# AvalonEnjoyer/pytorch-ViT-paper-replication

Measured on AMD Instinct MI355X. Metric: images/sec (whole node) ViT-B/16 224px bf16 at 1/2/4/8 MI355X, higher is better.
Workload: dtype bf16; 1 GPU; model=ViT-B/16, global_batch=256, per_gpu_batch=256, seq_len=197, image_size=224, parallelism=dp1, impl=fused, grad_transport=none, optimizer=Adam(wd=0.03 decay group) + clip 1.0 + warmup/linear-decay LR, dropout=0.1 (mlp, embedding)

## Files before the change

pytorch_vit_paper_replication_amd/csrc/attention.hip:

```cpp
#include "attn_common.h"
#include "kernels.h"

namespace pvr {
namespace {


template <int DH, bool DROP, int QG, int KT>
__global__ void __launch_bounds__(256) __attribute__((amdgpu_waves_per_eu(3))) attn_fwd_kernel(const uint16_t* __restrict__ qkv, int64_t ld, uint16_t* __restrict__ out,
                                                        int64_t ld_o, float* __restrict__ lse, int N, int H, int D, float scale,
                                                        AttnDrop drop, AttnQ8 q8) {
  using C = Hd<DH>;
  static_assert(KT == 32 || KT == 64, "keys per tile");
  constexpr int NFR = KT / 16;
  constexpr int TILE_BYTES = KT * 128 * C::NH;
  constexpr int QW = 16 * QG;
  extern __shared__ __attribute__((aligned(16))) char smem[];
  const int lane = threadIdx.x & 63;
  const int wave = __builtin_amdgcn_readfirstlane(threadIdx.x >> 6);
  const int g = lane >> 4, li = lane & 15;
  const int nqb = (N + 4 * QW - 1) / (4 * QW);
  const int L = xcd_remap(blockIdx.x, gridDim.x);
  const int bh = L / nqb, b = bh / H, h = bh % H;
  const int q0 = (L % nqb) * 4 * QW + wave * QW;

// ... 1760 lines not shown
}
PVR_DEV uint4 cls_pack8(const float (&f)[8]) {
  return make_uint4(pack2bf(f[0], f[1]), pack2bf(f[2], f[3]), pack2bf(f[4], f[5]), pack2bf(f[6], f[7]));
}
PVR_DEV float cls_dot8(const float (&a)[8], const float (&b)[8]) {
  float s = 0.f;
#pragma unroll
  for (int j = 0; j < 8; ++j) s = fmaf(a[j], b[j], s);
  return s;
}
template <int CH>
PVR_DEV float cls_group_sum(float v, int gbase) {
  if constexpr (CH == 8) {
    return oct_sum(v);
  } else if constexpr (CH == 16) {
    return row16_sum(v);
  } else {
    float t = 0.f;
#pragma unroll
    for (int j = 0; j < CH; ++j) t += __shfl(v, min(gbase + j, 63), 64);
    return t;
  }
}
template <bool MAX>
PVR_DEV float cls_block_reduce(float v, float* r4) {
  v = MAX ? wave_max(v) : wave_sum(v);
  __syncthreads();
  if ((threadIdx.x & 63) == 0) r4[threadIdx.x >> 6] = v;
  __syncthreads();
  return MAX ? fmaxf(fmaxf(r4[0], r4[1]), fmaxf(r4[2], r4[3])) : (r4[0] + r4[1]) + (r4[2] + r4[3]);
}

template <int DH>
__global__ void __launch_bounds__(256) attn_cls_fwd_kernel(const uint16_t* __restrict__ qkv, int64_t ld, uint16_t* __restrict__ out,
                                                            int64_t ld_o, float* __restrict__ lse, int N, int H, int D, float scale) {
  constexpr int CH = DH / 8, GPW = 64 / CH, NG = 4 * GPW;
  extern __shared__ float cls_sc[];
  __shared__ float gred[NG * DH];
  __shared__ float r4[4];
  const int bh = blockIdx.x, b = bh / H, h = bh % H;
  const int tid = threadIdx.x, lane = tid & 63, wave = tid >> 6;
  const int g = lane / CH, c = lane % CH;
  const bool act = g < GPW;
  const uint16_t* base = qkv + (int64_t)b * N * ld + h * DH + c * 8;
  float qf[8];
#pragma unroll
  for (int j = 0; j < 8; ++j) qf[j] = 0.f;
  if (act) cls_unpack8(*(const uint4*)base, qf);
  for (int k0 = wave * GPW; k0 < N; k0 += NG) {
    const int k = k0 + g;
    const bool live = act && k < N;
    float sv = 0.f;
    if (live) {
      float kf[8];
      cls_unpack8(*(const uint4*)(base + (int64_t)k * ld + D), kf);
      sv = cls_dot8(qf, kf);
    }
    sv = cls_group_sum<CH>(sv, g * CH);
    if (live && c == 0) cls_sc[k] = sv * scale;
  }
  __syncthreads();
  float m = -INFINITY;
  for (int k = tid; k < N; k += 256) m = fmaxf(m, cls_sc[k]);
  m = cls_block_reduce<true>(m, r4);
  float l = 0.f;
  for (int k = tid; k < N; k += 256) {
    const float pk = __builtin_amdgcn_exp2f((cls_sc[k] - m) * LOG2E);
    cls_sc[k] = pk;
    l += pk;
  }
  l = cls_block_reduce<false>(l, r4);
  if (tid == 0) lse[bh] = m + logf(l);
  float acc[8];
#pragma unroll
  for (int j = 0; j < 8; ++j) acc[j] = 0.f;
  if (act) {
    for (int k = wave * GPW + g; k < N; k += NG) {
      float vf[8];
      cls_unpack8(*(const uint4*)(base + (int64_t)k * ld + 2 * D), vf);
      const float pk = cls_sc[k];
#pragma unroll
      for (int j = 0; j < 8; ++j) acc[j] = fmaf(pk, vf[j], acc[j]);
    }
#pragma unroll
    for (int j = 0; j < 8; ++j) gred[(wave * GPW + g) * DH + c * 8 + j] = acc[j];
  }
  __syncthreads();
  if (tid < DH) {
    float o = 0.f;
#pragma unroll 4
    for (int gg = 0; gg < NG; ++gg) o += gred[gg * DH + tid];
    out[(int64_t)b * ld_o + h * DH + tid] = f2bf(o / l);
  }
}

template <int DH>
__global__ void __launch_bounds__(256) attn_cls_bwd_kernel(const uint16_t* __restrict__ qkv, int64_t ld, const uint16_t* __restrict__ o,
                                                            int64_t ld_o, const uint16_t* __restrict__ dout, int64_t ld_do,
                                                            const float* __restrict__ lse, uint16_t* __restrict__ dqkv, int64_t ld_dq,
                                                            float* __restrict__ dq0, int N, int H, int D, float scale) {
  constexpr int CH = DH / 8, GPW = 64 / CH, NG = 4 * GPW;
  __shared__ float gred[NG * DH];
  const int bh = blockIdx.x, b = bh / H, h = bh % H;
  const int tid = threadIdx.x, lane = tid & 63, wave = tid >> 6;
  const int g = lane / CH, c = lane % CH;
  const bool act = g < GPW;
  const int col = h * DH + c * 8;
  const uint16_t* base = qkv + (int64_t)b * N * ld + col;
  uint16_t* dbase = dqkv + (int64_t)b * N * ld_dq + col;
  float qf[8], dof[8], dqa[8];
#pragma unroll
  for (int j = 0; j < 8; ++j) qf[j] = dof[j] = dqa[j] = 0.f;
  float dpart = 0.f;
  if (act) {
    float of[8];
    cls_unpack8(*(const uint4*)base, qf);
    cls_unpack8(*(const uint4*)(dout + (int64_t)b * ld_do + col), dof);
    cls_unpack8(*(const uint4*)(o + (int64_t)b * ld_o + col), of);
    dpart = cls_dot8(dof, of);
  }
  const float delta = cls_group_sum<CH>(dpart, g * CH);
  const float l2 = lse[bh] * LOG2E, sl2 = scale * LOG2E;
  for (int k0 = wave * GPW; k0 < N; k0 += NG) {
    const int k = k0 + g;
    const bool live = act && k < N;
    float kf[8], vf[8];
    float sv = 0.f, tv = 0.f;
    if (live) {
      const uint4 kq = *(const uint4*)(base + (int64_t)k * ld + D);
      const uint4 vq = *(const uint4*)(base + (int64_t)k * ld + 2 * D);
      cls_unpack8(kq, kf);
      cls_unpack8(vq, vf);
      sv = cls_dot8(qf, kf);
      tv = cls_dot8(dof, vf);
    }
    sv = cls_group_sum<CH>(sv, g * CH);
    tv = cls_group_sum<CH>(tv, g * CH);
    if (live) {
      const float pk = __builtin_amdgcn_exp2f(sv * sl2 - l2);
      const float ds = pk * (tv - delta) * scale;
      float dk[8], dv[8];
#pragma unroll
      for (int j = 0; j < 8; ++j) {
        dv[j] = pk * dof[j];
        dk[j] = ds * qf[j];
        dqa[j] = fmaf(ds, kf[j], dqa[j]);
      }
      uint16_t* row = dbase + (int64_t)k * ld_dq;
      if (k > 0) *(uint4*)row = make_uint4(0u, 0u, 0u, 0u);
      *(uint4*)(row + D) = cls_pack8(dk);
      *(uint4*)(row + 2 * D) = cls_pack8(dv);
    }
  }
  if (act) {
#pragma unroll
    for (int j = 0; j < 8; ++j) gred[(wave * GPW + g) * DH + c * 8 + j] = dqa[j];
  }
  __syncthreads();
  if (tid < DH) {
    float dq = 0.f;
#pragma unroll 4
    for (int gg = 0; gg < NG; ++gg) dq += gred[gg * DH + tid];
    dqkv[(int64_t)b * N * ld_dq + h * DH + tid] = f2bf(dq);
    dq0[(int64_t)b * D + h * DH + tid] = dq;
  }
}

__global__ void __launch_bounds__(256) attn_cls_dbias_kernel(const float* __restrict__ dq0, const uint16_t* __restrict__ dout,
                                                              int64_t ld_do, float* __restrict__ dbias, int B, int D) {
  const int col = blockIdx.x * 256 + threadIdx.x;
  if (col >= D) return;
  float sq = 0.f, sv = 0.f;
#pragma unroll 8
  for (int b = 0; b < B; ++b) {
    sq += dq0[(int64_t)b * D + col];
    sv += bf2f(dout[(int64_t)b * ld_do + col]);
  }
  dbias[col] += sq;
  dbias[2 * D + col] += sv;
}

bool attn_cls_args_ok(int B, int N, int H, int D, int64_t ld, int64_t ld_o) {
  return B > 0 && N > 0 && H > 0 && D % H == 0 && pvr_attn_cls_ok(N, D / H) && ld % 8 == 0 && ld_o % 8 == 0 && ld >= 3 * (int64_t)D &&
         ld_o >= D;
}

}
}

extern "C" int pvr_attn_cls_ok(int N, int dh) { return N >= 1 && N <= 8192 && pvr_attn_head_dim_supported(dh) ? 1 : 0; }

extern "C" hipError_t pvr_attn_cls_fwd(const uint16_t* qkv, int64_t ld, uint16_t* out, int64_t ld_o, float* lse, int B, int N, int H,
                                       int D, float scale, hipStream_t s) {
  using namespace pvr;
  if (!attn_cls_args_ok(B, N, H, D, ld, ld_o)) return hipErrorInvalidValue;
  const dim3 grid(B * H), block(256);
  const size_t smem = (size_t)N * sizeof(float);
  switch (D / H) {
#define PVR_CLS_DH(DH) \
  case DH: hipLaunchKernelGGL(attn_cls_fwd_kernel<DH>, grid, block, smem, s, qkv, ld, out, ld_o, lse, N, H, D, scale); break;
    PVR_CLS_DH(64) PVR_CLS_DH(80) PVR_CLS_DH(96) PVR_CLS_DH(128)
#undef PVR_CLS_DH
    default: return hipErrorInvalidValue;
  }
  return hipGetLastError();
}

extern "C" hipError_t pvr_attn_cls_bwd(const uint16_t* qkv, int64_t ld, const uint16_t* o, int64_t ld_o, const uint16_t* dout,
                                       int64_t ld_do, const float* lse, uint16_t* dqkv, int64_t ld_dq, float* dq0, int B, int N, int H,
                                       int D, float scale, hipStream_t s) {
  using namespace pvr;
  if (!attn_cls_args_ok(B, N, H, D, ld, ld_o) || ld_do % 8 != 0 || ld_do < D || ld_dq % 8 != 0 || ld_dq < 3 * (int64_t)D)
    return hipErrorInvalidValue;
  const dim3 grid(B * H), block(256);
  switch (D / H) {
#define PVR_CLS_DH(DH) \
  case DH: hipLaunchKernelGGL(attn_cls_bwd_kernel<DH>, grid, block, 0, s, qkv, ld, o, ld_o, dout, ld_do, lse, dqkv, ld_dq, dq0, N, H, D, scale); break;
    PVR_CLS_DH(64) PVR_CLS_DH(80) PVR_CLS_DH(96) PVR_CLS_DH(128)
#undef PVR_CLS_DH
    default: return hipErrorInvalidValue;
  }
  return hipGetLastError();
}

extern "C" hipError_t pvr_attn_cls_dbias(const float* dq0, const uint16_t* dout, int64_t ld_do, float* dbias, int B, int D, hipStream_t s) {
  if (B <= 0 || D <= 0 || ld_do < D) return hipErrorInvalidValue;
  hipLaunchKernelGGL(pvr::attn_cls_dbias_kernel, dim3((D + 255) / 256), dim3(256), 0, s, dq0, dout, ld_do, dbias, B, D);
  return hipGetLastError();
}
```

pytorch_vit_paper_replication_amd/csrc/bindings.cpp:

```cpp
#include <cstdlib>
#include <algorithm>
#include <map>
#include <torch/extension.h>
#include <c10/hip/HIPStream.h>
#include <hip/hip_runtime.h>

#include "kernels.h"

namespace {

hipStream_t stream() { return c10::hip::getCurrentHIPStream().stream(); }
using ScratchKey = std::pair<int, int64_t>;
ScratchKey scratch_key(int dev) { return std::make_pair(dev, (int64_t)c10::hip::getCurrentHIPStream().id()); }
template <class T>
std::map<ScratchKey, T>& scratch_map() {
  static auto* m = new std::map<ScratchKey, T>();
  return *m;
}
struct SkCounters { torch::Tensor t; };
struct DetWs { torch::Tensor t; };
struct DqWs { torch::Tensor t; };
struct AttnWs { torch::Tensor t; };

int num_cus() {
// ... 1259 lines not shown
    else
      dbias->add_(dqkv.sum(0, false, torch::kFloat32));
  }
  return dqkv;
}

std::vector<torch::Tensor> attn_cls_fwd(torch::Tensor qkv, int64_t B, int64_t N, int64_t H, double scale) {
  TORCH_CHECK(qkv.dim() == 2 && qkv.size(0) == B * N && qkv.size(1) % 3 == 0 && H > 0, "attn_cls_fwd: qkv [B*N][3D]");
  const int64_t D = qkv.size(1) / 3;
  TORCH_CHECK(D % H == 0 && pvr_attn_cls_ok((int)N, (int)(D / H)), "attn_cls_fwd: unsupported N / head dim (attn_cls_ok)");
  auto out = torch::empty({B, D}, qkv.options());
  auto lse = torch::empty({B * H}, qkv.options().dtype(torch::kFloat32));
  check(pvr_attn_cls_fwd(bf(qkv, "qkv"), ld_of(qkv, "qkv"), bf_mut(out, "out"), D, f32_mut(lse, "lse"), (int)B, (int)N, (int)H, (int)D,
                         (float)scale, stream()),
        "attn_cls_fwd");
  return {out, lse};
}

std::vector<torch::Tensor> attn_cls_bwd(torch::Tensor dout, torch::Tensor qkv, torch::Tensor out, torch::Tensor lse, int64_t B, int64_t N,
                                        int64_t H, double scale) {
  TORCH_CHECK(qkv.dim() == 2 && qkv.size(0) == B * N && qkv.size(1) % 3 == 0 && H > 0, "attn_cls_bwd: qkv [B*N][3D]");
  const int64_t D = qkv.size(1) / 3;
  TORCH_CHECK(D % H == 0 && pvr_attn_cls_ok((int)N, (int)(D / H)), "attn_cls_bwd: unsupported N / head dim (attn_cls_ok)");
  TORCH_CHECK(dout.dim() == 2 && dout.size(0) == B && dout.size(1) == D && out.dim() == 2 && out.size(0) == B && out.size(1) == D &&
                  lse.numel() == B * H && lse.is_contiguous(),
              "attn_cls_bwd: dout / out [B][D], lse [B*H]");
  auto dqkv = torch::empty({B * N, 3 * D}, qkv.options());
  auto dq0 = torch::empty({B, D}, qkv.options().dtype(torch::kFloat32));
  check(pvr_attn_cls_bwd(bf(qkv, "qkv"), ld_of(qkv, "qkv"), bf(out, "out"), ld_of(out, "out"), bf(dout, "dout"), ld_of(dout, "dout"),
                         f32(lse, "lse"), bf_mut(dqkv, "dqkv"), 3 * D, f32_mut(dq0, "dq0"), (int)B, (int)N, (int)H, (int)D, (float)scale,
                         stream()),
        "attn_cls_bwd");
  return {dqkv, dq0};
}

void attn_cls_dbias(torch::Tensor dq0, torch::Tensor dout, torch::Tensor dbias) {
  TORCH_CHECK(dq0.dim() == 2 && dq0.is_contiguous() && dout.dim() == 2 && dout.size(0) == dq0.size(0) && dout.size(1) == dq0.size(1) &&
                  dbias.is_contiguous() && dbias.numel() == 3 * dq0.size(1),
              "attn_cls_dbias: dq0 f32 [B][D] contiguous, dout bf16 [B][D], dbias f32 [3D]");
  check(pvr_attn_cls_dbias(f32(dq0, "dq0"), bf(dout, "dout"), ld_of(dout, "dout"), f32_mut(dbias, "dbias"), (int)dq0.size(0),
                           (int)dq0.size(1), stream()),
        "attn_cls_dbias");
}

}

extern "C" const char* pvr_src_hash(void);

PYBIND11_MODULE(TORCH_EXTENSION_NAME, m) {
  m.doc() = "MI355X (gfx950) HIP kernels for pytorch_vit_paper_replication_amd";
  m.def("source_hash", []() { return std::string(pvr_src_hash()); },
        "content hash of the csrc/ sources this binary was built from (build.source_hash())");
  m.def("gemm_tail_split", [](int64_t M, int64_t N, int64_t K, int64_t elem_bytes, int64_t max_units) {
    return pvr_gemm_tail_split((int)M, (int)N, (int)K, (int)elem_bytes, (int)max_units); },
    py::arg("M"), py::arg("N"), py::arg("K"), py::arg("elem_bytes"), py::arg("max_units") = 0,
    "K-parts of the split tail round this GEMM shape gets (0: none)");
  m.def("set_attn_dbg", [](torch::Tensor t) { pvr_set_attn_dbg(t.defined() && t.numel() ? t.data_ptr() : nullptr); },
        "diagnostic builds (-DPVR_ATTN_STAMPS): int64 buffer for the attention backward's phase stamps "
        "[workgroup * waves + wave][8] (scripts/attn_stamps.py); a no-op otherwise");
  m.def("set_attn_prep_xcd", &pvr_set_attn_prep_xcd, "attention backward pre-pass: XCD-contiguous (batch, head) pairs (1) or round-robin (0, default); A/B");
  m.def("set_ln_fwd_q8_grid", &pvr_set_ln_fwd_q8_grid, "LayerNorm forward with the e4m3 copy: grid cap in workgroups per CU (A/B)");
  m.def("set_attn_fwd_head_qf", &pvr_set_attn_fwd_head_qf, "whole-head attention forward (dh 64, N <= 256): 16-query fragments per wave (1 = default, 2 = half the LDS reads with 7 waves; A/B)");
  m.def("set_attn_fwd_qg", &pvr_set_attn_fwd_qg, "tiled attention forward: 16-query groups per wave (0 = auto by query padding, 1 = round-3 form, 2 = forced; A/B)");
  m.def("set_fp8_persistent", &pvr_set_fp8_persistent, "fp8 fwd/dgrad GEMMs on the persistent ping-pong: 1 when the epilogue has no per-row input (default), 0 never (A/B)");
  m.def("set_deterministic", &set_deterministic, "deterministic reductions (partial rows + ordered sum) instead of float atomics");
  m.def("deterministic", &deterministic);
// ... 75 lines not shown
  m.def("scale_by", &scale_by);
  m.def("metrics_accum", &metrics_accum);
  m.def("rng_next", &rng_next);
  m.def("zero_f32", &zero_f32);
  m.def("gemm_fp8", &gemm_fp8, py::arg("A"), py::arg("fmt_a"), py::arg("B"), py::arg("fmt_b"), py::arg("C"), py::arg("M"),
        py::arg("N"), py::arg("K"), py::arg("epi"), py::arg("scale_a"), py::arg("scale_b"), py::arg("bias") = py::none(),
        py::arg("resid") = py::none(), py::arg("aux") = py::none(), py::arg("seed") = py::none(), py::arg("seed_offset") = 0,
        py::arg("drop_p") = 0.0, py::arg("colsum") = py::none(), py::arg("q_out") = py::none(), py::arg("q_scale") = py::none(),
        py::arg("q_amax") = py::none(), py::arg("q_fmt") = 0, py::arg("c_skip") = false, py::arg("tail_limit") = 0);
  m.def("fp8_transpose", &fp8_transpose);
  m.def("gemm_fp8_wgrad_mn", &gemm_fp8_wgrad_mn, py::arg("dy8"), py::arg("x8"), py::arg("ws"), py::arg("N"), py::arg("K"),
        py::arg("T"), py::arg("scale_a"), py::arg("scale_b"), py::arg("ksplit"), py::arg("fmt_a") = 1);
  m.def("fp8_quant", &fp8_quant, py::arg("x"), py::arg("y"), py::arg("qscale"), py::arg("amax"), py::arg("fmt"));
  m.def("fp8_dequant", &fp8_dequant, py::arg("x"), py::arg("dscale") = py::none(), py::arg("fmt") = 0);
  m.def("fp8_scale_update", &fp8_scale_update);
  m.def("fp8_quant_t", &fp8_quant_t);
  m.def("gemm_fp8_wgrad", &gemm_fp8_wgrad, py::arg("A8"), py::arg("B8"), py::arg("ws"), py::arg("N"), py::arg("K"), py::arg("Tp"),
        py::arg("scale_a"), py::arg("scale_b"), py::arg("ksplit"), py::arg("fmt_a") = 1);
  m.def("fp8_quant_multi", &fp8_quant_multi, py::arg("segs"), py::arg("nchunks"), py::arg("qscale"), py::arg("amax"), py::arg("fmt"),
        py::arg("amax_only"));
  m.def("attn_fwd", &attn_fwd, py::arg("qkv"), py::arg("B"), py::arg("N"), py::arg("H"), py::arg("scale"),
        py::arg("seed") = py::none(), py::arg("seed_offset") = 0, py::arg("drop_p") = 0.0, py::arg("q_out") = py::none(),
        py::arg("q_scale") = py::none(), py::arg("q_amax") = py::none(), py::arg("q_only") = false);
  m.def("attn_bwd", &attn_bwd, py::arg("dout"), py::arg("qkv"), py::arg("out"), py::arg("lse"), py::arg("B"), py::arg("N"),
        py::arg("H"), py::arg("scale"), py::arg("dbias") = py::none(), py::arg("dbias_part") = py::none(),
        py::arg("seed") = py::none(), py::arg("seed_offset") = 0, py::arg("drop_p") = 0.0, py::arg("q_out") = py::none(),
        py::arg("q_scale") = py::none(), py::arg("q_amax") = py::none(), py::arg("q_only") = false,
        py::arg("q_fmt") = 1);
  m.def("attn_cls_ok", [](int64_t N, int64_t dh) { return pvr_attn_cls_ok((int)N, (int)dh) != 0; },
        "the class-token attention kernels take this token count and head dim");
  m.def("attn_cls_fwd", &attn_cls_fwd, py::arg("qkv"), py::arg("B"), py::arg("N"), py::arg("H"), py::arg("scale"));
  m.def("attn_cls_bwd", &attn_cls_bwd, py::arg("dout"), py::arg("qkv"), py::arg("out"), py::arg("lse"), py::arg("B"), py::arg("N"),
        py::arg("H"), py::arg("scale"));
  m.def("attn_cls_dbias", &attn_cls_dbias);
  m.def("attn_bwd_q8_ok", &attn_bwd_q8_ok, "attn_bwd can write dQKV's e5m2 copy for this shape");
  m.def("arch", []() { return std::string("gfx950"); });
}
```

pytorch_vit_paper_replication_amd/csrc/kernels.h:

```cpp
#pragma once
#include <stdint.h>

#include <hip/hip_runtime_api.h>

#include "gemm_params.h"

namespace pvr {

struct AdamGroup {
  float lr, beta1, beta2, eps, weight_decay;
  float bc1, bc2_sqrt;
  int decoupled;
  float one_minus_beta1, one_minus_beta2;
};
constexpr int ADAM_GROUP_COLS = 10;
static_assert(sizeof(AdamGroup) == ADAM_GROUP_COLS * sizeof(float), "AdamGroup is one float32 [10] row of the group table");

struct AdamEma {
  float* buf = nullptr; const float* pair = nullptr; float decay = 0.f, one_minus_decay = 1.f;
};

constexpr int LAMB_ALWAYS_ADAPT = 2;
constexpr int LAMB_CHUNK = 4096;

// ... 144 lines not shown
                         unsigned* amax, int fmt, hipStream_t s);
hipError_t pvr_fp8_quant_multi(const int64_t* segs, int nseg, int64_t nchunks, const float* qscale, unsigned* amax, int fmt,
                               int amax_only, hipStream_t s);
hipError_t pvr_fp8_quant_t(const uint16_t* x, int64_t ldx, uint8_t* y, int64_t ldy, int T, int C, const float* qscale, int fmt,
                           hipStream_t s);
hipError_t pvr_fp8_transpose(const uint8_t* x, int64_t ldx, uint8_t* y, int64_t ldy, int T, int C, hipStream_t s);
hipError_t pvr_fp8_dequant(const uint8_t* x, float* y, int64_t n, const float* dscale, int fmt, hipStream_t s);
hipError_t pvr_fp8_scale_update(float* hist, int H, unsigned* amax, float* qscale, float* dscale, const float* fmax, int s0, int s1,
                                float margin_mul, hipStream_t s);

void pvr_set_attn_fwd_qg(int qg);
void pvr_set_attn_fwd_head_qf(int qf);
void pvr_set_attn_prep_xcd(int on);
void pvr_set_attn_dbg(void* p);
int pvr_attn_head_dim_supported(int dh);
hipError_t pvr_attn_fwd(const uint16_t* qkv, int64_t ld, uint16_t* out, int64_t ld_o, float* lse, int B, int N, int H, int D,
                        float scale, pvr::DropSite drop, pvr::Fp8Copy q8, int q8_only, hipStream_t s);
int pvr_attn_dbias_splits(int B, int NQ);
hipError_t pvr_attn_dbias_reduce(const float* part, float* ws, float* dbias, int B, int H, int NQ, int D, hipStream_t s);
int pvr_attn_bwd_waves(int N);
int pvr_attn_bwd_key_blocks(int N);
int pvr_attn_bwd_needs_dq_acc(int N, int dh, int dbias, int drop, int det);
int64_t pvr_attn_bwd_ws_floats(int B, int N, int H, int D, int dbias, int drop, int det);
int pvr_attn_bwd_q8_ok(int N, int drop);
int pvr_attn_bwd_uses_pipe(int B, int N, int H, int D, int64_t ld, int64_t ld_do, int64_t ld_o, int64_t ld_dq, int drop);
int pvr_attn_bwd_part_rows(int B, int N, int H, int D, int64_t ld, int64_t ld_do, int64_t ld_o, int64_t ld_dq, int drop);
hipError_t pvr_attn_bwd(const pvr::AttnBwdParams* p, hipStream_t s);
int pvr_attn_cls_ok(int N, int dh);
hipError_t pvr_attn_cls_fwd(const uint16_t* qkv, int64_t ld, uint16_t* out, int64_t ld_o, float* lse, int B, int N, int H, int D,
                            float scale, hipStream_t s);
hipError_t pvr_attn_cls_bwd(const uint16_t* qkv, int64_t ld, const uint16_t* o, int64_t ld_o, const uint16_t* dout, int64_t ld_do,
                            const float* lse, uint16_t* dqkv, int64_t ld_dq, float* dq0, int B, int N, int H, int D, float scale,
                            hipStream_t s);
hipError_t pvr_attn_cls_dbias(const float* dq0, const uint16_t* dout, int64_t ld_do, float* dbias, int B, int D, hipStream_t s);

}
```

pytorch_vit_paper_replication_amd/ops/fused_vit.py:

```python
from __future__ import annotations

import math
from typing import List, Optional

import torch
import torch.nn.functional as F

from .. import _ext
from . import gemm

SITE_SHIFT = 32
ATTN_SITE = 1 << 20
DROP_PATH_SITE = 1 << 21
PATCH_DROP_SITE = 1 << 22
ERASE_SITE = 1 << 23


DGRAD_TAP = None


def site_drop(seed: Optional[torch.Tensor], site: int, p: float, training: bool):
    if seed is None or not training or p <= 0.0:
        return None
    return (seed, site << SITE_SHIFT, float(p))
# ... 409 lines not shown
        if q8res is not None:
            pre_q[3] = q8res
        elif fp8_qkv:
            prod = f8d[0].grad_producer(f8d[1], 3)
            if side_db and prod is not None:
                pre_q[3] = gemm.bias_grad(dqkv, gbqkv, quant=prod)
                side_db = False
            else:
                pre_q[3] = f8d[0].grad_quant(dqkv, f8d[1], 3)
        store.on_side(attn_wgrads, dz1, o, dqkv, xn1, do, *(() if db_part is None else (db_part,)), *side8(2, 3))
        dxn1 = dgrad(dqkv, wqkv, 3)
        dx = torch.empty_like(dx2)
        if prev is not None:
            seed, soff, p = gemm._drop_args(prev.drop2)
            dp_kw = gemm._drop_path_kw(_dp(prev.dp2, N))
            dzp = torch.empty_like(dx2) if seed is not None or dp_kw else None
            pf8 = (f8d[0], f8d[1] - 1) if f8d is not None and f8d[1] > 0 else None
            q_kw, q_dz = _ln_grad_quant(pf8, 0, dx.shape, dx.device)
            dz_nostore = (q_dz is not None and dzp is not None and T >= 256 and DGRAD_TAP is None
                          and prev.w2 is not None and store.bf16_t(prev.w2) is not None
                          and pf8[0].wgrad_ready(pf8[1], 0, 3))
            ext.layernorm_bwd(dxn1, D, x, D, mean1, rstd1, ln1w, dx1, D, dx, D, g(ln1w), g(ln1b), T,
                              dsum=g(prev.b2), dz=dzp, seed=seed, seed_offset=soff, drop_p=p, dz_nostore=dz_nostore, **dp_kw, **q_kw)
            if dzp is not None:
                _poison(dzp, dz_nostore)
            prev.dz2, prev.dz2_q, prev.done = dzp, q_dz, True
        else:
            ext.layernorm_bwd(dxn1, D, x, D, mean1, rstd1, ln1w, dx1, D, dx, D, g(ln1w), g(ln1b), T)
        store.grad_ready([bo, wo, bqkv, wqkv, ln1w, ln1b])
        return (dx,) + (None,) * (9 + len(params))


CLS_LAST_BLOCK = True


def cls_last_block_ok(N: int, H: int, D: int, f8, dropa) -> bool:
    return (CLS_LAST_BLOCK and f8 is None and gemm._drop_args(dropa)[0] is None
            and D % H == 0 and bool(_ext.ext().attn_cls_ok(N, D // H)))


class EncoderBlockClsFn(torch.autograd.Function):

    @staticmethod
    def forward(ctx, x, B, N, H, eps1, eps2, store, drops, links, *params):
        ext = _ext.ext()
        drop1, drop2, _, dpa, dpm = _split_drops(drops)
        ln1w, ln1b, wqkv, bqkv, wo, bo, ln2w, ln2b, w1, b1, w2, b2 = params
        T, D = x.shape
        ctx.links = links if links is not None else (None, None)
        M = w1.shape[0]
        scale = 1.0 / math.sqrt(D // H)
        need_bwd = getattr(store, "grad_enabled", True) and any(ctx.needs_input_grad)
        xn1, mean1, rstd1 = ext.layernorm_fwd(x, ln1w, ln1b, eps1, T, D)
        qkv = gemm.linear_fwd(xn1, store.bf16(wqkv), bqkv)
        o, lse = ext.attn_cls_fwd(qkv, B, N, H, scale)
        xc = x.view(B, N, D)[:, 0]
        x1 = gemm.linear_fwd(o, store.bf16(wo), bo, resid=xc, drop_path=_dp(dpa, 1))
        xn2, mean2, rstd2 = ext.layernorm_fwd(x1, ln2w, ln2b, eps2, B, D)
        u = torch.empty(B, M, dtype=torch.bfloat16, device=x.device) if need_bwd else None
        h = gemm.linear_fwd(xn2, store.bf16(w1), b1, gelu_aux=u, gelu=True, drop=drop1, drop_row_mul=N)
        x2 = gemm.linear_fwd(h, store.bf16(w2), b2, resid=x1, drop=drop2, drop_row_mul=N, drop_path=_dp(dpm, 1))
        if need_bwd:
            ctx.save_for_backward(x, xn1, mean1, rstd1, qkv, o, lse, x1, xn2, mean2, rstd2, u, h)
        ctx.meta = (B, N, H, scale, store, drop2, params)
        ctx.dpath = (dpa, dpm)
        return x2

    @staticmethod
    def backward(ctx, dx2):
        ext = _ext.ext()
        det = _ext.deterministic()
        x, xn1, mean1, rstd1, qkv, o, lse, x1, xn2, mean2, rstd2, u, h = ctx.saved_tensors
        B, N, H, scale, store, drop2, params = ctx.meta
        dpa, dpm = ctx.dpath
        ln1w, ln1b, wqkv, bqkv, wo, bo, ln2w, ln2b, w1, b1, w2, b2 = params
        g = store.grad_dest
        dx2 = dx2.contiguous()
        T, D = x.shape
        _, prev = ctx.links

        def dgrad(dy, w, which, dgelu_aux=None, colsum=None):
            out = gemm.linear_dgrad(dy, store.bf16(w), dgelu_aux=dgelu_aux, wt=store.bf16_t(w), colsum=colsum)
            if DGRAD_TAP is not None:
                DGRAD_TAP(which, out)
            return out

        if drop2 is not None or dpm is not None:
            dz2 = torch.empty_like(dx2)
            gemm.bias_grad(dx2, g(b2), drop=drop2, dz=dz2, row_mul=N, drop_path=_dp(dpm, 1))
        else:
            dz2 = dx2
            if b2.requires_grad:
                gemm.bias_grad(dx2, g(b2))
        gb1 = g(b1)
        gw2, gw1 = g(w2), g(w1)
        du = dgrad(dz2, w2, 0, dgelu_aux=u, colsum=None if det else gb1)
        if det and gb1 is not None:
            gemm.bias_grad(du, gb1)

        def mlp_wgrads():
            if gw2 is not None:
                gemm.linear_wgrad(dz2, h, gw2)
            if gw1 is not None:
                gemm.linear_wgrad(du, xn2, gw1)

        store.on_side(mlp_wgrads, dz2, h, du, xn2)
        dxn2 = dgrad(du, w1, 1)
        dx1 = torch.empty_like(dx2)
        dz1 = torch.empty_like(dx1) if dpa is not None else dx1
        ext.layernorm_bwd(dxn2, D, x1, D, mean2, rstd2, ln2w, dx2, D, dx1, D, g(ln2w), g(ln2b), B, dsum=g(bo),
                          **(dict(dz=dz1, **gemm._drop_path_kw(_dp(dpa, 1))) if dpa is not None else {}))
        store.grad_ready([w2, b2, w1, b1, ln2w, ln2b])
        gwo, gwqkv, gbqkv = g(wo), g(wqkv), g(bqkv)
        do = dgrad(dz1, wo, 2)
        dqkv, dq0 = ext.attn_cls_bwd(do, qkv, o, lse, B, N, H, scale)

        def attn_wgrads():
            if gbqkv is not None:
                ext.attn_cls_dbias(dq0, do, gbqkv.view(-1))
            if gwo is not None:
                gemm.linear_wgrad(dz1, o, gwo)
            if gwqkv is not None:
                gemm.linear_wgrad(dqkv, xn1, gwqkv)

        store.on_side(attn_wgrads, dz1, o, dqkv, xn1, do, dq0)
        dxn1 = dgrad(dqkv, wqkv, 3)
        dx = torch.empty_like(x)
        if prev is not None:
            seed, soff, p = gemm._drop_args(prev.drop2)
            dp_kw = gemm._drop_path_kw(_dp(prev.dp2, N))
            dzp = torch.empty_like(x) if seed is not None or dp_kw else None
            ext.layernorm_bwd(dxn1, D, x, D, mean1, rstd1, ln1w, dx1, D, dx, D, g(ln1w), g(ln1b), T,
                              dsum=g(prev.b2), dz=dzp, seed=seed, seed_offset=soff, drop_p=p, dres_every=N, **dp_kw)
            prev.dz2, prev.dz2_q, prev.done = dzp, None, True
        else:
            ext.layernorm_bwd(dxn1, D, x, D, mean1, rstd1, ln1w, dx1, D, dx, D, g(ln1w), g(ln1b), T, dres_every=N)
        store.grad_ready([bo, wo, bqkv, wqkv, ln1w, ln1b])
        return (dx,) + (None,) * (8 + len(params))


class HeadFn(torch.autograd.Function):

    @staticmethod
    def forward(ctx, tokens, B, N, eps, store, ln_w, ln_b, head_w, head_b):
        ext = _ext.ext()
        logits, xhat, rstd = ext.head_fwd(tokens, B, N, ln_w, ln_b, eps, head_w, head_b)
        ctx.save_for_backward(xhat, rstd)
        ctx.meta = (B, N, store, ln_w, ln_b, head_w, head_b)
        return logits

    @staticmethod
    def backward(ctx, dlogits):
        ext = _ext.ext()
        _ext.deterministic()
        xhat, rstd = ctx.saved_tensors
        B, N, store, ln_w, ln_b, head_w, head_b = ctx.meta
        g = store.grad_dest
        dlogits = dlogits.float().contiguous()
        dtokens = ext.head_bwd(dlogits, xhat, rstd, ln_w, ln_b, head_w, B, N, g(head_w), g(head_b), g(ln_w), g(ln_b))
# ... 139 lines not shown
```

pytorch_vit_paper_replication_amd/ops/gemm.py:

```python
from __future__ import annotations

import math
from typing import Optional, Tuple

import torch

from .. import _ext

EPI_BF16, EPI_GELU, EPI_DGELU, EPI_F32_ATOMIC, EPI_F32_STORE = range(5)



def _n_cus() -> int:
    global _N_CUS
    if _N_CUS is None:
        _N_CUS = torch.cuda.get_device_properties(torch.cuda.current_device()).multi_processor_count if torch.cuda.is_available() else 256
    return _N_CUS


_N_CUS = None
FORCE_TILE: Optional[int] = None

Drop = Optional[Tuple[torch.Tensor, int, float]]

# ... 69 lines not shown
    seed, soff, p = _drop_args(drop)
    epi = EPI_GELU if (gelu or gelu_aux is not None) else EPI_BF16
    if drop_path is not None and drop_path[2] <= 0.0:
        drop_path = None
    if drop_path is not None and (resid is None or epi != EPI_BF16 or addend is not None or row_remap[0]):
        raise ValueError("drop_path needs the residual epilogue (resid given; no GELU, addend or row_remap)")
    if drop_row_mul > 1 and p > 0.0:
        if addend is not None or row_remap[0]:
            raise ValueError("drop_row_mul does not combine with addend / row_remap")
        _gemm(x, True, w, True, out, T, N, K, epi, bias, resid, None, 0, gelu_aux, 0, 0, 0, seed, soff, p, 0,
              tile=0, drop_row_mul=int(drop_row_mul), drop_path=drop_path)
        return out
    S = _small_splitk(T, N, K) if (p == 0.0 and gelu_aux is None and addend is None and row_remap[0] == 0
                                   and drop_path is None) else 0
    if S:
        ksplit = math.ceil(math.ceil(K / S) / 64) * 64
        nsplit = math.ceil(K / ksplit)
        ws = _workspace(nsplit * T * N, x.device)[:nsplit * T * N].view(nsplit, T, N)
        ext = _ext.ext()
        ext.gemm(x, True, w, True, ws, T, N, K, EPI_F32_STORE, None, None, None, 0, None, 0, 0, 0, None, 0, 0.0, ksplit, 14)
        ext.splitk_epilogue(ws, nsplit, out, bias, resid, epi == EPI_GELU)
        return out
    kind = "gelu" if epi == EPI_GELU else "resid" if resid is not None else "bias"
    tile = _tile(T, N, K, "fwd")
    if addend is None and row_remap[0] == 0 and drop_path is None:
        tile = _ws_tile(kind, tile)
    _gemm(x, True, w, True, out, T, N, K, epi, bias, resid, addend, addend_period, gelu_aux,
          row_remap[0], row_remap[1], row_remap[2], seed, soff, p, 0, tile=tile, drop_path=drop_path)
    return out


def linear_dgrad(dy: torch.Tensor, w: torch.Tensor, *, dgelu_aux: Optional[torch.Tensor] = None,
                 drop: Drop = None, out: Optional[torch.Tensor] = None, wt: Optional[torch.Tensor] = None,
                 colsum: Optional[torch.Tensor] = None, tile: Optional[int] = None) -> torch.Tensor:
    T, N = dy.shape
    K = w.shape[1]
    if out is None:
        out = torch.empty(T, K, dtype=torch.bfloat16, device=dy.device)
    seed, soff, p = None, 0, 0.0
    epi = EPI_DGELU if dgelu_aux is not None else EPI_BF16
    if colsum is not None and dgelu_aux is None:
        raise ValueError("colsum is fused only into the GELU-backward epilogue")
    if wt is not None and N % 64 == 0:
        _gemm(dy, True, wt, True, out, T, K, N, epi, None, None, None, 0, dgelu_aux, 0, 0, 0,
              seed, soff, p, 0, tile=_ws_tile("dgelu" if dgelu_aux is not None else "dgrad", _tile(T, K, N, "dgrad_t")),
              colsum=colsum, tail_limit=DGRAD_TAIL_UNITS)
    else:
        _ext.ext().gemm(dy, True, w, False, out, T, K, N, epi, None, None, None, 0, dgelu_aux, 0, 0, 0,
                        seed, soff, p, 0, _tile(T, K, N, "dgrad") if tile is None else tile, colsum=colsum,
                        tail_limit=DGRAD_TAIL_UNITS)
    return out


_WGRAD_WGS = 256
_WGRAD_WGS_NARROW = 144
OVERLAPPED = False


def wgrad_splits(T: int, N: int, K: int, tile: int = 0) -> int:
    if tile == 12:
        tiles = math.ceil(N / 256) * math.ceil(K / 256)
        wgs = _WGRAD_WGS_NARROW if OVERLAPPED and min(N, K) <= 768 else _WGRAD_WGS
        return max(1, min(wgs // tiles, max(1, T // 256)))
    tiles = math.ceil(N / 128) * math.ceil(K / 128)
    target = 1024
    s = max(1, round(target / tiles))
    s = min(s, max(1, T // 512))
    return s


SPLITK_FIXUP = _os.environ.get("PVR_SPLITK_FIXUP", "0") != "0"
_cus = None


def _num_cus() -> int:
    global _cus
    if _cus is None:
        _cus = int(_ext.ext().num_cus())
    return _cus


# ... 60 lines not shown
```

Baseline: 7951 images/sec.

## Compute only CLS query row in last block's QKV projection

```diff
diff --git a/pytorch_vit_paper_replication_amd/csrc/attention.hip b/pytorch_vit_paper_replication_amd/csrc/attention.hip
--- a/pytorch_vit_paper_replication_amd/csrc/attention.hip
+++ b/pytorch_vit_paper_replication_amd/csrc/attention.hip
@@ -1816,8 +1816,9 @@
 }
 
 template <int DH>
-__global__ void __launch_bounds__(256) attn_cls_fwd_kernel(const uint16_t* __restrict__ qkv, int64_t ld, uint16_t* __restrict__ out,
-                                                            int64_t ld_o, float* __restrict__ lse, int N, int H, int D, float scale) {
+__global__ void __launch_bounds__(256) attn_cls_fwd_kernel(const uint16_t* __restrict__ q, int64_t ld_q0, const uint16_t* __restrict__ kp,
+                                                            const uint16_t* __restrict__ vp, int64_t ld, uint16_t* __restrict__ out,
+                                                            int64_t ld_o, float* __restrict__ lse, int N, int H, float scale) {
   constexpr int CH = DH / 8, GPW = 64 / CH, NG = 4 * GPW;
   extern __shared__ float cls_sc[];
   __shared__ float gred[NG * DH];
@@ -1826,18 +1827,20 @@
   const int tid = threadIdx.x, lane = tid & 63, wave = tid >> 6;
   const int g = lane / CH, c = lane % CH;
   const bool act = g < GPW;
-  const uint16_t* base = qkv + (int64_t)b * N * ld + h * DH + c * 8;
+  const int64_t tok0 = (int64_t)b * N * ld + h * DH + c * 8;
+  const uint16_t* kbase = kp + tok0;
+  const uint16_t* vbase = vp + tok0;
   float qf[8];
 #pragma unroll
   for (int j = 0; j < 8; ++j) qf[j] = 0.f;
-  if (act) cls_unpack8(*(const uint4*)base, qf);
+  if (act) cls_unpack8(*(const uint4*)(q + (int64_t)b * ld_q0 + h * DH + c * 8), qf);
   for (int k0 = wave * GPW; k0 < N; k0 += NG) {
     const int k = k0 + g;
     const bool live = act && k < N;
     float sv = 0.f;
     if (live) {
       float kf[8];
-      cls_unpack8(*(const uint4*)(base + (int64_t)k * ld + D), kf);
+      cls_unpack8(*(const uint4*)(kbase + (int64_t)k * ld), kf);
       sv = cls_dot8(qf, kf);
     }
     sv = cls_group_sum<CH>(sv, g * CH);
@@ -1861,7 +1864,7 @@
   if (act) {
     for (int k = wave * GPW + g; k < N; k += NG) {
       float vf[8];
-      cls_unpack8(*(const uint4*)(base + (int64_t)k * ld + 2 * D), vf);
+      cls_unpack8(*(const uint4*)(vbase + (int64_t)k * ld), vf);
       const float pk = cls_sc[k];
 #pragma unroll
       for (int j = 0; j < 8; ++j) acc[j] = fmaf(pk, vf[j], acc[j]);
@@ -1878,10 +1881,12 @@
   }
 }
 
-template <int DH>
-__global__ void __launch_bounds__(256) attn_cls_bwd_kernel(const uint16_t* __restrict__ qkv, int64_t ld, const uint16_t* __restrict__ o,
+template <int DH, bool QROWS>
+__global__ void __launch_bounds__(256) attn_cls_bwd_kernel(const uint16_t* __restrict__ q, int64_t ld_q0, const uint16_t* __restrict__ kp,
+                                                            const uint16_t* __restrict__ vp, int64_t ld, const uint16_t* __restrict__ o,
                                                             int64_t ld_o, const uint16_t* __restrict__ dout, int64_t ld_do,
-                                                            const float* __restrict__ lse, uint16_t* __restrict__ dqkv, int64_t ld_dq,
+                                                            const float* __restrict__ lse, uint16_t* __restrict__ dqp, int64_t ld_dq0,
+                                                            uint16_t* __restrict__ dkp, uint16_t* __restrict__ dvp, int64_t ld_dq,
                                                             float* __restrict__ dq0, int N, int H, int D, float scale) {
   constexpr int CH = DH / 8, GPW = 64 / CH, NG = 4 * GPW;
   __shared__ float gred[NG * DH];
@@ -1890,15 +1895,16 @@
   const int g = lane / CH, c = lane % CH;
   const bool act = g < GPW;
   const int col = h * DH + c * 8;
-  const uint16_t* base = qkv + (int64_t)b * N * ld + col;
-  uint16_t* dbase = dqkv + (int64_t)b * N * ld_dq + col;
+  const uint16_t* kbase = kp + (int64_t)b * N * ld + col;
+  const uint16_t* vbase = vp + (int64_t)b * N * ld + col;
+  const int64_t dtok0 = (int64_t)b * N * ld_dq + col;
   float qf[8], dof[8], dqa[8];
 #pragma unroll
   for (int j = 0; j < 8; ++j) qf[j] = dof[j] = dqa[j] = 0.f;
   float dpart = 0.f;
   if (act) {
     float of[8];
-    cls_unpack8(*(const uint4*)base, qf);
+    cls_unpack8(*(const uint4*)(q + (int64_t)b * ld_q0 + col), qf);
     cls_unpack8(*(const uint4*)(dout + (int64_t)b * ld_do + col), dof);
     cls_unpack8(*(const uint4*)(o + (int64_t)b * ld_o + col), of);
     dpart = cls_dot8(dof, of);
@@ -1911,8 +1917,8 @@
     float kf[8], vf[8];
     float sv = 0.f, tv = 0.f;
     if (live) {
-      const uint4 kq = *(const uint4*)(base + (int64_t)k * ld + D);
-      const uint4 vq = *(const uint4*)(base + (int64_t)k * ld + 2 * D);
+      const uint4 kq = *(const uint4*)(kbase + (int64_t)k * ld);
+      const uint4 vq = *(const uint4*)(vbase + (int64_t)k * ld);
       cls_unpack8(kq, kf);
       cls_unpack8(vq, vf);
       sv = cls_dot8(qf, kf);
@@ -1930,10 +1936,12 @@
         dk[j] = ds * qf[j];
         dqa[j] = fmaf(ds, kf[j], dqa[j]);
       }
-      uint16_t* row = dbase + (int64_t)k * ld_dq;
-      if (k > 0) *(uint4*)row = make_uint4(0u, 0u, 0u, 0u);
-      *(uint4*)(row + D) = cls_pack8(dk);
-      *(uint4*)(row + 2 * D) = cls_pack8(dv);
+      const int64_t row = dtok0 + (int64_t)k * ld_dq;
+      if constexpr (QROWS) {
+        if (k > 0) *(uint4*)(dqp + row) = make_uint4(0u, 0u, 0u, 0u);
+      }
+      *(uint4*)(dkp + row) = cls_pack8(dk);
+      *(uint4*)(dvp + row) = cls_pack8(dv);
     }
   }
   if (act) {
@@ -1945,7 +1953,7 @@
     float dq = 0.f;
 #pragma unroll 4
     for (int gg = 0; gg < NG; ++gg) dq += gred[gg * DH + tid];
-    dqkv[(int64_t)b * N * ld_dq + h * DH + tid] = f2bf(dq);
+    dqp[(QROWS ? (int64_t)b * N * ld_dq : (int64_t)b * ld_dq0) + h * DH + tid] = f2bf(dq);
     dq0[(int64_t)b * D + h * DH + tid] = dq;
   }
 }
@@ -1964,9 +1972,43 @@
   dbias[2 * D + col] += sv;
 }
 
-bool attn_cls_args_ok(int B, int N, int H, int D, int64_t ld, int64_t ld_o) {
-  return B > 0 && N > 0 && H > 0 && D % H == 0 && pvr_attn_cls_ok(N, D / H) && ld % 8 == 0 && ld_o % 8 == 0 && ld >= 3 * (int64_t)D &&
+bool attn_cls_args_ok(int B, int N, int H, int D, int64_t ld, int64_t ld_o, int slices = 3) {
+  return B > 0 && N > 0 && H > 0 && D % H == 0 && pvr_attn_cls_ok(N, D / H) && ld % 8 == 0 && ld_o % 8 == 0 && ld >= slices * (int64_t)D &&
          ld_o >= D;
+}
+bool attn_cls_row_ok(const void* ptr, int64_t ld, int D) { return ptr != nullptr && ld % 8 == 0 && ld >= D; }
+
+hipError_t attn_cls_fwd_launch(const uint16_t* q, int64_t ld_q0, const uint16_t* kp, const uint16_t* vp, int64_t ld, uint16_t* out,
+                               int64_t ld_o, float* lse, int B, int N, int H, int D, float scale, hipStream_t s) {
+  const dim3 grid(B * H), block(256);
+  const size_t smem = (size_t)N * sizeof(float);
+  switch (D / H) {
+#define PVR_CLS_DH(DH) \
+  case DH: hipLaunchKernelGGL(attn_cls_fwd_kernel<DH>, grid, block, smem, s, q, ld_q0, kp, vp, ld, out, ld_o, lse, N, H, scale); break;
+    PVR_CLS_DH(64) PVR_CLS_DH(80) PVR_CLS_DH(96) PVR_CLS_DH(128)
+#undef PVR_CLS_DH
+    default: return hipErrorInvalidValue;
+  }
+  return hipGetLastError();
+}
+
+template <bool QROWS>
+hipError_t attn_cls_bwd_launch(const uint16_t* q, int64_t ld_q0, const uint16_t* kp, const uint16_t* vp, int64_t ld, const uint16_t* o,
+                               int64_t ld_o, const uint16_t* dout, int64_t ld_do, const float* lse, uint16_t* dqp, int64_t ld_dq0,
+                               uint16_t* dkp, uint16_t* dvp, int64_t ld_dq, float* dq0, int B, int N, int H, int D, float scale,
+                               hipStream_t s) {
+  const dim3 grid(B * H), block(256);
+  switch (D / H) {
+#define PVR_CLS_DH(DH)                                                                                                                 \
+  case DH:                                                                                                                             \
+    hipLaunchKernelGGL((attn_cls_bwd_kernel<DH, QROWS>), grid, block, 0, s, q, ld_q0, kp, vp, ld, o, ld_o, dout, ld_do, lse, dqp, ld_dq0, \
+                       dkp, dvp, ld_dq, dq0, N, H, D, scale);                                                                          \
+    break;
+    PVR_CLS_DH(64) PVR_CLS_DH(80) PVR_CLS_DH(96) PVR_CLS_DH(128)
+#undef PVR_CLS_DH
+    default: return hipErrorInvalidValue;
+  }
+  return hipGetLastError();
 }
 
 }
@@ -1978,16 +2020,14 @@
                                        int D, float scale, hipStream_t s) {
   using namespace pvr;
   if (!attn_cls_args_ok(B, N, H, D, ld, ld_o)) return hipErrorInvalidValue;
-  const dim3 grid(B * H), block(256);
-  const size_t smem = (size_t)N * sizeof(float);
-  switch (D / H) {
-#define PVR_CLS_DH(DH) \
-  case DH: hipLaunchKernelGGL(attn_cls_fwd_kernel<DH>, grid, block, smem, s, qkv, ld, out, ld_o, lse, N, H, D, scale); break;
-    PVR_CLS_DH(64) PVR_CLS_DH(80) PVR_CLS_DH(96) PVR_CLS_DH(128)
-#undef PVR_CLS_DH
-    default: return hipErrorInvalidValue;
-  }
-  return hipGetLastError();
+  return attn_cls_fwd_launch(qkv, (int64_t)N * ld, qkv + D, qkv + 2 * D, ld, out, ld_o, lse, B, N, H, D, scale, s);
+}
+
+extern "C" hipError_t pvr_attn_cls_fwd_kv(const uint16_t* q0, int64_t ld_q0, const uint16_t* kv, int64_t ld_kv, uint16_t* out,
+                                          int64_t ld_o, float* lse, int B, int N, int H, int D, float scale, hipStream_t s) {
+  using namespace pvr;
+  if (!attn_cls_args_ok(B, N, H, D, ld_kv, ld_o, 2) || !attn_cls_row_ok(q0, ld_q0, D)) return hipErrorInvalidValue;
+  return attn_cls_fwd_launch(q0, ld_q0, kv, kv + D, ld_kv, out, ld_o, lse, B, N, H, D, scale, s);
 }
 
 extern "C" hipError_t pvr_attn_cls_bwd(const uint16_t* qkv, int64_t ld, const uint16_t* o, int64_t ld_o, const uint16_t* dout,
@@ -1996,15 +2036,20 @@
   using namespace pvr;
   if (!attn_cls_args_ok(B, N, H, D, ld, ld_o) || ld_do % 8 != 0 || ld_do < D || ld_dq % 8 != 0 || ld_dq < 3 * (int64_t)D)
     return hipErrorInvalidValue;
-  const dim3 grid(B * H), block(256);
-  switch (D / H) {
-#define PVR_CLS_DH(DH) \
-  case DH: hipLaunchKernelGGL(attn_cls_bwd_kernel<DH>, grid, block, 0, s, qkv, ld, o, ld_o, dout, ld_do, lse, dqkv, ld_dq, dq0, N, H, D, scale); break;
-    PVR_CLS_DH(64) PVR_CLS_DH(80) PVR_CLS_DH(96) PVR_CLS_DH(128)
-#undef PVR_CLS_DH
-    default: return hipErrorInvalidValue;
-  }
-  return hipGetLastError();
+  return attn_cls_bwd_launch<true>(qkv, (int64_t)N * ld, qkv + D, qkv + 2 * D, ld, o, ld_o, dout, ld_do, lse, dqkv, 0, dqkv + D,
+                                   dqkv + 2 * D, ld_dq, dq0, B, N, H, D, scale, s);
+}
+
+extern "C" hipError_t pvr_attn_cls_bwd_kv(const uint16_t* q0, int64_t ld_q0, const uint16_t* kv, int64_t ld_kv, const uint16_t* o,
+                                          int64_t ld_o, const uint16_t* dout, int64_t ld_do, const float* lse, uint16_t* dkv,
+                                          int64_t ld_dkv, float* dq0, uint16_t* dq0_bf, int64_t ld_dq0, int B, int N, int H, int D,
+                                          float scale, hipStream_t s) {
+  using namespace pvr;
+  if (!attn_cls_args_ok(B, N, H, D, ld_kv, ld_o, 2) || !attn_cls_row_ok(q0, ld_q0, D) || !attn_cls_row_ok(dout, ld_do, D) ||
+      !attn_cls_row_ok(dq0_bf, ld_dq0, D) || dkv == nullptr || dq0 == nullptr || ld_dkv % 8 != 0 || ld_dkv < 2 * (int64_t)D)
+    return hipErrorInvalidValue;
+  return attn_cls_bwd_launch<false>(q0, ld_q0, kv, kv + D, ld_kv, o, ld_o, dout, ld_do, lse, dq0_bf, ld_dq0, dkv, dkv + D, ld_dkv, dq0,
+                                    B, N, H, D, scale, s);
 }
 
 extern "C" hipError_t pvr_attn_cls_dbias(const float* dq0, const uint16_t* dout, int64_t ld_do, float* dbias, int B, int D, hipStream_t s) {
diff --git a/pytorch_vit_paper_replication_amd/csrc/bindings.cpp b/pytorch_vit_paper_replication_amd/csrc/bindings.cpp
--- a/pytorch_vit_paper_replication_amd/csrc/bindings.cpp
+++ b/pytorch_vit_paper_replication_amd/csrc/bindings.cpp
@@ -1315,6 +1315,41 @@
                          stream()),
         "attn_cls_bwd");
   return {dqkv, dq0};
+}
+
+void check_cls_kv(const torch::Tensor& q0, const torch::Tensor& kv, int64_t B, int64_t N, int64_t H, const char* what) {
+  TORCH_CHECK(kv.dim() == 2 && kv.size(0) == B * N && kv.size(1) % 2 == 0 && H > 0, what, ": kv [B*N][2D]");
+  const int64_t D = kv.size(1) / 2;
+  TORCH_CHECK(q0.dim() == 2 && q0.size(0) == B && q0.size(1) == D, what, ": q0 [B][D]");
+  TORCH_CHECK(D % H == 0 && pvr_attn_cls_ok((int)N, (int)(D / H)), what, ": unsupported N / head dim (attn_cls_ok)");
+}
+
+std::vector<torch::Tensor> attn_cls_fwd_kv(torch::Tensor q0, torch::Tensor kv, int64_t B, int64_t N, int64_t H, double scale) {
+  check_cls_kv(q0, kv, B, N, H, "attn_cls_fwd_kv");
+  const int64_t D = kv.size(1) / 2;
+  auto out = torch::empty({B, D}, kv.options());
+  auto lse = torch::empty({B * H}, kv.options().dtype(torch::kFloat32));
+  check(pvr_attn_cls_fwd_kv(bf(q0, "q0"), ld_of(q0, "q0"), bf(kv, "kv"), ld_of(kv, "kv"), bf_mut(out, "out"), D, f32_mut(lse, "lse"),
+                            (int)B, (int)N, (int)H, (int)D, (float)scale, stream()),
+        "attn_cls_fwd_kv");
+  return {out, lse};
+}
+
+std::vector<torch::Tensor> attn_cls_bwd_kv(torch::Tensor dout, torch::Tensor q0, torch::Tensor kv, torch::Tensor out, torch::Tensor lse,
+                                           int64_t B, int64_t N, int64_t H, double scale) {
+  check_cls_kv(q0, kv, B, N, H, "attn_cls_bwd_kv");
+  const int64_t D = kv.size(1) / 2;
+  TORCH_CHECK(dout.dim() == 2 && dout.size(0) == B && dout.size(1) == D && out.dim() == 2 && out.size(0) == B && out.size(1) == D &&
+                  lse.numel() == B * H && lse.is_contiguous(),
+              "attn_cls_bwd_kv: dout / out [B][D], lse [B*H]");
+  auto dkv = torch::empty({B * N, 2 * D}, kv.options());
+  auto dq0 = torch::empty({B, D}, kv.options().dtype(torch::kFloat32));
+  auto dq0_bf = torch::empty({B, D}, kv.options());
+  check(pvr_attn_cls_bwd_kv(bf(q0, "q0"), ld_of(q0, "q0"), bf(kv, "kv"), ld_of(kv, "kv"), bf(out, "out"), ld_of(out, "out"),
+                            bf(dout, "dout"), ld_of(dout, "dout"), f32(lse, "lse"), bf_mut(dkv, "dkv"), 2 * D, f32_mut(dq0, "dq0"),
+                            bf_mut(dq0_bf, "dq0_bf"), D, (int)B, (int)N, (int)H, (int)D, (float)scale, stream()),
+        "attn_cls_bwd_kv");
+  return {dkv, dq0, dq0_bf};
 }
 
 void attn_cls_dbias(torch::Tensor dq0, torch::Tensor dout, torch::Tensor dbias) {
@@ -1456,6 +1491,9 @@
   m.def("attn_cls_fwd", &attn_cls_fwd, py::arg("qkv"), py::arg("B"), py::arg("N"), py::arg("H"), py::arg("scale"));
   m.def("attn_cls_bwd", &attn_cls_bwd, py::arg("dout"), py::arg("qkv"), py::arg("out"), py::arg("lse"), py::arg("B"), py::arg("N"),
         py::arg("H"), py::arg("scale"));
+  m.def("attn_cls_fwd_kv", &attn_cls_fwd_kv, py::arg("q0"), py::arg("kv"), py::arg("B"), py::arg("N"), py::arg("H"), py::arg("scale"));
+  m.def("attn_cls_bwd_kv", &attn_cls_bwd_kv, py::arg("dout"), py::arg("q0"), py::arg("kv"), py::arg("out"), py::arg("lse"), py::arg("B"),
+        py::arg("N"), py::arg("H"), py::arg("scale"));
   m.def("attn_cls_dbias", &attn_cls_dbias);
   m.def("attn_bwd_q8_ok", &attn_bwd_q8_ok, "attn_bwd can write dQKV's e5m2 copy for this shape");
   m.def("arch", []() { return std::string("gfx950"); });
diff --git a/pytorch_vit_paper_replication_amd/csrc/kernels.h b/pytorch_vit_paper_replication_amd/csrc/kernels.h
--- a/pytorch_vit_paper_replication_amd/csrc/kernels.h
+++ b/pytorch_vit_paper_replication_amd/csrc/kernels.h
@@ -200,6 +200,11 @@
 hipError_t pvr_attn_cls_bwd(const uint16_t* qkv, int64_t ld, const uint16_t* o, int64_t ld_o, const uint16_t* dout, int64_t ld_do,
                             const float* lse, uint16_t* dqkv, int64_t ld_dq, float* dq0, int B, int N, int H, int D, float scale,
                             hipStream_t s);
+hipError_t pvr_attn_cls_fwd_kv(const uint16_t* q0, int64_t ld_q0, const uint16_t* kv, int64_t ld_kv, uint16_t* out, int64_t ld_o,
+                               float* lse, int B, int N, int H, int D, float scale, hipStream_t s);
+hipError_t pvr_attn_cls_bwd_kv(const uint16_t* q0, int64_t ld_q0, const uint16_t* kv, int64_t ld_kv, const uint16_t* o, int64_t ld_o,
+                               const uint16_t* dout, int64_t ld_do, const float* lse, uint16_t* dkv, int64_t ld_dkv, float* dq0,
+                               uint16_t* dq0_bf, int64_t ld_dq0, int B, int N, int H, int D, float scale, hipStream_t s);
 hipError_t pvr_attn_cls_dbias(const float* dq0, const uint16_t* dout, int64_t ld_do, float* dbias, int B, int D, hipStream_t s);
 
 }
diff --git a/pytorch_vit_paper_replication_amd/ops/fused_vit.py b/pytorch_vit_paper_replication_amd/ops/fused_vit.py
--- a/pytorch_vit_paper_replication_amd/ops/fused_vit.py
+++ b/pytorch_vit_paper_replication_amd/ops/fused_vit.py
@@ -465,6 +465,7 @@
 
 
 CLS_LAST_BLOCK = True
+CLS_QUERY_ROWS = True
 
 
 def cls_last_block_ok(N: int, H: int, D: int, f8, dropa) -> bool:
@@ -485,8 +486,14 @@
         scale = 1.0 / math.sqrt(D // H)
         need_bwd = getattr(store, "grad_enabled", True) and any(ctx.needs_input_grad)
         xn1, mean1, rstd1 = ext.layernorm_fwd(x, ln1w, ln1b, eps1, T, D)
-        qkv = gemm.linear_fwd(xn1, store.bf16(wqkv), bqkv)
-        o, lse = ext.attn_cls_fwd(qkv, B, N, H, scale)
+        w16 = store.bf16(wqkv)
+        if CLS_QUERY_ROWS:
+            qkv = gemm.linear_fwd(xn1, w16[D:], bqkv[D:])
+            q0 = gemm.linear_fwd(xn1.view(B, N, D)[:, 0], w16[:D], bqkv[:D])
+            o, lse = ext.attn_cls_fwd_kv(q0, qkv, B, N, H, scale)
+        else:
+            qkv, q0 = gemm.linear_fwd(xn1, w16, bqkv), None
+            o, lse = ext.attn_cls_fwd(qkv, B, N, H, scale)
         xc = x.view(B, N, D)[:, 0]
         x1 = gemm.linear_fwd(o, store.bf16(wo), bo, resid=xc, drop_path=_dp(dpa, 1))
         xn2, mean2, rstd2 = ext.layernorm_fwd(x1, ln2w, ln2b, eps2, B, D)
@@ -494,7 +501,7 @@
         h = gemm.linear_fwd(xn2, store.bf16(w1), b1, gelu_aux=u, gelu=True, drop=drop1, drop_row_mul=N)
         x2 = gemm.linear_fwd(h, store.bf16(w2), b2, resid=x1, drop=drop2, drop_row_mul=N, drop_path=_dp(dpm, 1))
         if need_bwd:
-            ctx.save_for_backward(x, xn1, mean1, rstd1, qkv, o, lse, x1, xn2, mean2, rstd2, u, h)
+            ctx.save_for_backward(x, xn1, mean1, rstd1, qkv, o, lse, x1, xn2, mean2, rstd2, u, h, q0)
         ctx.meta = (B, N, H, scale, store, drop2, params)
         ctx.dpath = (dpa, dpm)
         return x2
@@ -503,7 +510,7 @@
     def backward(ctx, dx2):
         ext = _ext.ext()
         det = _ext.deterministic()
-        x, xn1, mean1, rstd1, qkv, o, lse, x1, xn2, mean2, rstd2, u, h = ctx.saved_tensors
+        x, xn1, mean1, rstd1, qkv, o, lse, x1, xn2, mean2, rstd2, u, h, q0 = ctx.saved_tensors
         B, N, H, scale, store, drop2, params = ctx.meta
         dpa, dpm = ctx.dpath
         ln1w, ln1b, wqkv, bqkv, wo, bo, ln2w, ln2b, w1, b1, w2, b2 = params
@@ -546,18 +553,32 @@
         store.grad_ready([w2, b2, w1, b1, ln2w, ln2b])
         gwo, gwqkv, gbqkv = g(wo), g(wqkv), g(bqkv)
         do = dgrad(dz1, wo, 2)
-        dqkv, dq0 = ext.attn_cls_bwd(do, qkv, o, lse, B, N, H, scale)
+        if q0 is not None:
+            dqkv, dq0, dq0_bf = ext.attn_cls_bwd_kv(do, q0, qkv, o, lse, B, N, H, scale)
+        else:
+            (dqkv, dq0), dq0_bf = ext.attn_cls_bwd(do, qkv, o, lse, B, N, H, scale), None
 
         def attn_wgrads():
             if gbqkv is not None:
                 ext.attn_cls_dbias(dq0, do, gbqkv.view(-1))
             if gwo is not None:
                 gemm.linear_wgrad(dz1, o, gwo)
-            if gwqkv is not None:
+            if gwqkv is not None and q0 is not None:
+                gemm.linear_wgrad(dqkv, xn1, gwqkv[D:])
+                gemm.linear_wgrad(dq0_bf, xn1.view(B, N, D)[:, 0], gwqkv[:D])
+            elif gwqkv is not None:
                 gemm.linear_wgrad(dqkv, xn1, gwqkv)
 
-        store.on_side(attn_wgrads, dz1, o, dqkv, xn1, do, dq0)
-        dxn1 = dgrad(dqkv, wqkv, 3)
+        store.on_side(attn_wgrads, dz1, o, dqkv, xn1, do, dq0, *(() if q0 is None else (dq0_bf,)))
+        if q0 is not None:
+            w16, wt = store.bf16(wqkv), store.bf16_t(wqkv)
+            dxn1 = gemm.linear_dgrad(dqkv, w16[D:], wt=None if wt is None else wt[:, D:])
+            dxc = dxn1.view(B, N, D)[:, 0]
+            gemm.linear_dgrad(dq0_bf, w16[:D], wt=None if wt is None else wt[:, :D], resid=dxc, out=dxc)
+            if DGRAD_TAP is not None:
+                DGRAD_TAP(3, dxn1)
+        else:
+            dxn1 = dgrad(dqkv, wqkv, 3)
         dx = torch.empty_like(x)
         if prev is not None:
             seed, soff, p = gemm._drop_args(prev.drop2)
diff --git a/pytorch_vit_paper_replication_amd/ops/gemm.py b/pytorch_vit_paper_replication_amd/ops/gemm.py
--- a/pytorch_vit_paper_replication_amd/ops/gemm.py
+++ b/pytorch_vit_paper_replication_amd/ops/gemm.py
@@ -125,7 +125,8 @@
 
 def linear_dgrad(dy: torch.Tensor, w: torch.Tensor, *, dgelu_aux: Optional[torch.Tensor] = None,
                  drop: Drop = None, out: Optional[torch.Tensor] = None, wt: Optional[torch.Tensor] = None,
-                 colsum: Optional[torch.Tensor] = None, tile: Optional[int] = None) -> torch.Tensor:
+                 colsum: Optional[torch.Tensor] = None, tile: Optional[int] = None,
+                 resid: Optional[torch.Tensor] = None) -> torch.Tensor:
     T, N = dy.shape
     K = w.shape[1]
     if out is None:
@@ -134,12 +135,16 @@
     epi = EPI_DGELU if dgelu_aux is not None else EPI_BF16
     if colsum is not None and dgelu_aux is None:
         raise ValueError("colsum is fused only into the GELU-backward epilogue")
+    if resid is not None and dgelu_aux is not None:
+        raise ValueError("resid does not combine with the GELU-backward epilogue")
     if wt is not None and N % 64 == 0:
-        _gemm(dy, True, wt, True, out, T, K, N, epi, None, None, None, 0, dgelu_aux, 0, 0, 0,
-              seed, soff, p, 0, tile=_ws_tile("dgelu" if dgelu_aux is not None else "dgrad", _tile(T, K, N, "dgrad_t")),
+        kind = "dgelu" if dgelu_aux is not None else "resid" if resid is not None else "dgrad"
+        inplace = resid is not None and resid.data_ptr() == out.data_ptr()
+        _gemm(dy, True, wt, True, out, T, K, N, epi, None, resid, None, 0, dgelu_aux, 0, 0, 0,
+              seed, soff, p, 0, tile=0 if inplace else _ws_tile(kind, _tile(T, K, N, "dgrad_t")),
               colsum=colsum, tail_limit=DGRAD_TAIL_UNITS)
     else:
-        _ext.ext().gemm(dy, True, w, False, out, T, K, N, epi, None, None, None, 0, dgelu_aux, 0, 0, 0,
+        _ext.ext().gemm(dy, True, w, False, out, T, K, N, epi, None, resid, None, 0, dgelu_aux, 0, 0, 0,
                         seed, soff, p, 0, _tile(T, K, N, "dgrad") if tile is None else tile, colsum=colsum,
                         tail_limit=DGRAD_TAIL_UNITS)
     return out
```

After: 7973 images/sec (median of 6 runs). About the same (+0.3%).
